# davxy/ark-ec-vrfs

Hardware: AMD Instinct MI355X
Metric: Bandersnatch IETF-ECVRF verifies/sec, 2^20 batch per GPU (higher is better)
Workload: dtype u32; 1 GPU; IETF ECVRF verify, Bandersnatch_SHA-512_ELL2, batch 2^20 per GPU, compressed points (161 B/verify), checked decode: on curve + prime-order subgroup, as arkworks' deserialisation, ad="", about 1 in 16 proofs forged (BASELINE.json configs[2]); global_batch=1048576, parallelism=items sharded x1, result gather only, subgroup_check=True

## Files before the change

ark_ec_vrfs_amd/csrc/api.hip:

```cpp
#include "../../include/vrfhip.h"

#include <hip/hip_runtime.h>

#include <algorithm>
#include <cstdio>
#include <cstdlib>
#include <cstring>
#include <memory>
#include <mutex>
#include <string>
#include <thread>
#include <vector>

#include "kernels.h"
#include "digest.cuh"
#include "msm.cuh"
#include "msm_g1.h"
#include "p256.h"
#include "bsw.h"
#include "constants_bsw.gen.h"

namespace vrf {
size_t pairing_oct_lines_bytes(size_t items);
void launch_pairing_check2_oct_split(size_t n, const uint8_t* g1, const uint8_t* g2, size_t g2_stride, uint8_t* status, void* ws,
// ... 131 lines not shown
  int prev = -1;
  bool ok = true;
  explicit DeviceGuard(int dev) {
    if (hipGetDevice(&prev) != hipSuccess) prev = -1;
    if (prev != dev) ok = hipSetDevice(dev) == hipSuccess;
  }
  ~DeviceGuard() {
    if (prev >= 0) (void)hipSetDevice(prev);
  }
};

int32_t alloc_workspace(vrfhip_ctx* ctx, size_t cap) {
  if (ctx->d_ws) {
    HIP_TRY(hipFree(ctx->d_ws));
    ctx->d_ws = nullptr;
    ctx->ws_cap = 0;
    ctx->ws_bytes = 0;
  }
  if (ctx->sw) {
    const size_t total = p256::ws_bytes(cap);
    HIP_TRY(hipMalloc(&ctx->d_ws, total));
    ctx->p256_ws = p256::ws_carve(ctx->d_ws, cap);
    ctx->ws_cap = cap;
    ctx->ws_bytes = total;
    return VRFHIP_SUCCESS;
  }
  size_t tabs_b = cap * WS_TABS * WIN_TABLE_WORDS * sizeof(uint32_t);
  size_t pts_b = cap * PROVE_PTS_WORDS * sizeof(uint32_t);
  size_t aux_b = cap * AUX_WORDS * sizeof(uint32_t);
  size_t flags_b = (cap + 255) & ~size_t(255);
  size_t total = tabs_b + pts_b + aux_b + flags_b;
  HIP_TRY(hipMalloc(&ctx->d_ws, total));
  uint8_t* p = static_cast<uint8_t*>(ctx->d_ws);
  ctx->ws.tabs = reinterpret_cast<uint32_t*>(p); p += tabs_b;
  ctx->ws.pts = reinterpret_cast<uint32_t*>(p); p += pts_b;
  ctx->ws.aux = reinterpret_cast<uint32_t*>(p); p += aux_b;
  ctx->ws.flags = p;
  ctx->ws_cap = cap;
  ctx->ws_bytes = total;
  return VRFHIP_SUCCESS;
}

int32_t ensure_workspace(vrfhip_ctx* ctx, size_t items) {
  size_t want = std::min(items, ctx->chunk_limit);
  if (want <= ctx->ws_cap) return VRFHIP_SUCCESS;
  return alloc_workspace(ctx, want);
}

int32_t ensure_stage(vrfhip_ctx* ctx, size_t bytes) {
  if (bytes <= ctx->stage_bytes) return VRFHIP_SUCCESS;
  if (ctx->d_stage) {
    HIP_TRY(hipMemset(ctx->d_stage, 0, ctx->stage_bytes));
    HIP_TRY(hipFree(ctx->d_stage));
    ctx->d_stage = nullptr;
    ctx->stage_bytes = 0;
  }
  HIP_TRY(hipMalloc(&ctx->d_stage, bytes));
  ctx->stage_bytes = bytes;
  return VRFHIP_SUCCESS;
}

int32_t ensure_msm_workspace(vrfhip_ctx* ctx, size_t need) {
  if (need <= ctx->msm_ws_bytes) return VRFHIP_SUCCESS;
  if (ctx->d_msm_ws) HIP_TRY(hipFree(ctx->d_msm_ws));
  ctx->d_msm_ws = nullptr;
  ctx->msm_ws_bytes = 0;
// ... 2996 lines not shown
```

ark_ec_vrfs_amd/csrc/fr.cuh:

```cuda
#pragma once
#include "fe.cuh"

VRF_NS_BEGIN

template <class C>
VRF_HD void fr_montmul(uint32_t out[8], const uint32_t a[8], const uint32_t b[8]) {
  uint32_t t[10];
#pragma unroll
  for (int i = 0; i < 10; ++i) t[i] = 0;
#pragma unroll
  for (int i = 0; i < 8; ++i) {
    uint64_t c = 0;
#pragma unroll
    for (int j = 0; j < 8; ++j) {
      uint64_t x = (uint64_t)a[j] * b[i] + t[j] + c;
      t[j] = (uint32_t)x;
      c = x >> 32;
    }
    uint64_t x = (uint64_t)t[8] + c;
    t[8] = (uint32_t)x;
    t[9] = (uint32_t)(x >> 32);
    uint32_t m = t[0] * C::R_NINV32;
    c = ((uint64_t)m * C::r32(0) + t[0]) >> 32;
#pragma unroll
// ... 187 lines not shown
  acc5_muladd(v2, c2, vrfk::BS_GLV_B2_MAG, !(vrfk::BS_GLV_C2_NEG ^ vrfk::BS_GLV_B2_NEG));
  k1 = glv_finish(v1);
  k2 = glv_finish(v2);
}
#endif

VRF_HD void scalar_recode_signed4_128(uint32_t out[4], const uint32_t k[4]) {
  uint32_t c = 0;
#pragma unroll
  for (int i = 0; i < 4; ++i) {
    uint64_t x = (uint64_t)k[i] + 0x88888888u + c;
    out[i] = (uint32_t)x;
    c = (uint32_t)(x >> 32);
  }
}
VRF_HD int scalar_digit4_128(const uint32_t rec[4], int w) {
  uint32_t word = rec[0];
#pragma unroll
  for (int i = 1; i < 4; ++i)
    if ((w >> 3) == i) word = rec[i];
  return (int)((word >> ((w & 7) * 4)) & 15u) - 8;
}

constexpr uint32_t GLV_HALF_TOP_WORD_CAP = 0x77777777u;
static_assert(GLV_HALF_TOP_WORD_CAP < 0x80000000u, "bit 127 of a GLV half must be clear: the joint ladders start at bit 126");

VRF_HD int scalar_bit_128(const uint32_t k[4], int bit) {
  uint32_t word = k[0];
#pragma unroll
  for (int i = 1; i < 4; ++i)
    if ((bit >> 5) == i) word = k[i];
  return (int)((word >> (bit & 31)) & 1u);
}
VRF_HD void scalar_recode_signed2_128(uint32_t out[4], const uint32_t k[4]) {
  uint32_t c = 0;
#pragma unroll
  for (int i = 0; i < 4; ++i) {
    uint64_t x = (uint64_t)k[i] + 0x55555555u + c;
    out[i] = (uint32_t)x;
    c = (uint32_t)(x >> 32);
  }
}
VRF_HD int scalar_digit2_128(const uint32_t rec[4], int w) {
  uint32_t word = rec[0];
#pragma unroll
  for (int i = 1; i < 4; ++i)
    if ((w >> 4) == i) word = rec[i];
  return (int)((word >> ((w & 15) * 2)) & 3u) - 1;
}

VRF_NS_END
```

ark_ec_vrfs_amd/csrc/k_verify.hip:

```cpp
#include "kernels.h"
#include "tai_find.cuh"

VRF_NS_BEGIN


template <class S, int MINW>
__global__ void __launch_bounds__(BLOCK, MINW) k_verify_decode(VerifyArgs a) {
  size_t first = ((size_t)blockIdx.x * BLOCK + threadIdx.x) * a.k_decode;
  if (first >= a.n) return;
  verify_decode_multi<S, 3, false, S::HAS_GLV>(a.k_decode, a.T, first, a.n, a.pk, a.h, a.gamma, a.ws.tabs, a.ws.pts, a.ws.flags,
                                               a.check_mask, a.c, a.s);
}

template <class S>
__global__ void __launch_bounds__(BLOCK, 2) k_verify_input_from_alpha(size_t n, BytesView msg, uint8_t* enc, uint32_t* tabs,
                                                                      DevTables T, const uint8_t* tai_ctr) {
  size_t i = (size_t)blockIdx.x * BLOCK + threadIdx.x;
  if (i >= n) return;
  const uint8_t* m; uint32_t len;
  bytes_get(msg, i, m, len);
  PtE h = data_to_point<S>(m, len, T.sq, tai_ctr ? tai_ctr[i] : 0u);
  FeN x, y;
  te_to_affine(x, y, h);
  uint32_t e[8];
  te_encode_affine(e, x, y, T.sq.str.flags);
  store32(enc, i, e);
  if constexpr (S::HAS_GLV) jt_park_xy(tabs + i * (VERIFY_TABS * WIN_TABLE_WORDS) + JT_HXY, x, y);
  else build_glv_tables<S>(tabs + i * (VERIFY_TABS * WIN_TABLE_WORDS) + 2 * WIN_TABLE_WORDS, x, y);
}
template <class S, int MINW>
__global__ void __launch_bounds__(BLOCK, MINW) k_verify_decode_skip_h(VerifyArgs a) {
  size_t first = ((size_t)blockIdx.x * BLOCK + threadIdx.x) * a.k_decode;
  if (first >= a.n) return;
  verify_decode_multi<S, 2, true, S::HAS_GLV>(a.k_decode, a.T, first, a.n, a.pk, nullptr, a.gamma, a.ws.tabs, a.ws.pts,
                                              a.ws.flags, a.check_mask, a.c, a.s);
}

template <class S, int MINW>
__global__ void __launch_bounds__(BLOCK, MINW) k_verify_decode_keyed(VerifyArgs a) {
  size_t first = ((size_t)blockIdx.x * BLOCK + threadIdx.x) * a.k_decode;
  if (first >= a.n) return;
  verify_decode_multi<S, 2, false, S::HAS_GLV>(a.k_decode, a.T, first, a.n, nullptr, a.h, a.gamma, a.ws.tabs, a.ws.pts,
                                               a.ws.flags, a.check_mask, a.c, a.s);
#pragma unroll 1
  for (int k = 0; k < a.k_decode; ++k) {
    const size_t i = first + k;
    if (i >= a.n) break;
    const uint32_t key = a.key_index[i];
    const bool key_ok = key < a.n_keys && a.key_valid[key] != 0;
    if (!key_ok) a.ws.flags[i] = 0;
  }
}

template <class S>
__global__ void __launch_bounds__(BLOCK) k_verify_comb_u(VerifyArgs a) {
  size_t i = (size_t)blockIdx.x * BLOCK + threadIdx.x;
  if (i >= a.n) return;
  uint32_t c[8], s[8];
  load32(c, a.c, i); load32(s, a.s, i);
  load_cs_reduced<S>(c, s);
  const uint32_t key = a.key_index[i] < a.n_keys ? a.key_index[i] : 0;
  PtE r = gcomb_mul<S>(a.T.g_comb, s);
  r = comb_add<S>(r, a.key_combs + (size_t)key * COMB_WORDS, c, true);
  uint32_t* out = a.ws.pts + i * PROVE_PTS_WORDS;
  fe_store(out, r.X); fe_store(out + NL, r.Y); fe_store(out + 2 * NL, r.Z);
}

template <class S>
__global__ void __launch_bounds__(BLOCK) k_verify_decode_affine(VerifyArgs a) {
  size_t i = (size_t)blockIdx.x * BLOCK + threadIdx.x;
  if (i >= a.n) return;
  uint32_t xy[3][16], enc[3][8];
  const uint32_t* p0 = reinterpret_cast<const uint32_t*>(a.pk + i * 64);
  const uint32_t* p1 = reinterpret_cast<const uint32_t*>(a.h + i * 64);
  const uint32_t* p2 = reinterpret_cast<const uint32_t*>(a.gamma + i * 64);
#pragma unroll
  for (int j = 0; j < 16; ++j) { xy[0][j] = p0[j]; xy[1][j] = p1[j]; xy[2][j] = p2[j]; }
  uint32_t c[8], s[8];
  if constexpr (S::HAS_GLV) {
    load32(c, a.c, i); load32(s, a.s, i);
    load_cs_reduced<S>(c, s);
  }
  bool ok = verify_decode_affine_item<S, S::HAS_GLV>(enc, xy, a.ws.tabs + i * (VERIFY_TABS * WIN_TABLE_WORDS), a.T.sq,
                                                     a.check_mask, a.affine_in == 2, c, s);
  uint32_t* aux = a.ws.aux + i * AUX_WORDS;
#pragma unroll
  for (int j = 0; j < 8; ++j) { aux[j] = enc[0][j]; aux[8 + j] = enc[1][j]; aux[16 + j] = enc[2][j]; }
  a.ws.flags[i] = ok ? 1 : 0;
}

template <class S, int HALF>
__global__ void __launch_bounds__(BLOCK) k_verify_straus(VerifyArgs a) {
  size_t i = (size_t)blockIdx.x * BLOCK + threadIdx.x;
  if (i >= a.n) return;
  uint32_t c[8], s[8];
  load32(c, a.c, i); load32(s, a.s, i);
  load_cs_reduced<S>(c, s);
  uint32_t* out = a.ws.pts + i * PROVE_PTS_WORDS + HALF * UV_WORDS;
  const uint32_t* tabs = a.ws.tabs + i * (VERIFY_TABS * WIN_TABLE_WORDS);
  if constexpr (S::HAS_GLV) verify_joint_item<S, HALF>(out, a.T, tabs, c, s);
  else verify_straus_item<S, HALF>(out, a.T, tabs, c, s);
}

template <class S>
__global__ void __launch_bounds__(BLOCK) k_verify_straus_both(VerifyArgs a) {
  size_t i = (size_t)blockIdx.x * BLOCK + threadIdx.x;
  if (i >= a.n) return;
  uint32_t c[8], s[8];
  load32(c, a.c, i); load32(s, a.s, i);
  load_cs_reduced<S>(c, s);
  const uint32_t* tabs = a.ws.tabs + i * (VERIFY_TABS * WIN_TABLE_WORDS);
  if constexpr (S::HAS_GLV) {
    if (blockIdx.y == 0) verify_joint_item<S, 1>(a.ws.pts + i * PROVE_PTS_WORDS + UV_WORDS, a.T, tabs, c, s);
    else verify_joint_item<S, 0>(a.ws.pts + i * PROVE_PTS_WORDS, a.T, tabs, c, s);
  } else {
    if (blockIdx.y == 0) verify_straus_item<S, 1>(a.ws.pts + i * PROVE_PTS_WORDS + UV_WORDS, a.T, tabs, c, s);
    else verify_straus_item<S, 0>(a.ws.pts + i * PROVE_PTS_WORDS, a.T, tabs, c, s);
  }
}

template <class S, int MINW>
__global__ void __launch_bounds__(BLOCK, MINW) k_verify_finish(VerifyArgs a) {
  size_t first = ((size_t)blockIdx.x * BLOCK + threadIdx.x) * a.k_lane;
  if (first >= a.n) return;
  verify_finish_multi<S>(a.k_lane, first, a.n, a.ws.pts, PROVE_PTS_WORDS, a.pk, a.h, a.gamma,
                         a.affine_in ? a.ws.aux : nullptr, AUX_WORDS, a.c, a.s, a.ad, a.ws.flags, a.status,
                         a.T.sq.str, a.key_index, a.n_keys);
}

template <class S>
static void launch_verify_t(const VerifyArgs& a_in, hipStream_t st, hipEvent_t* ev) {
  VerifyArgs a = a_in;
  if (a.k_decode <= 0) a.k_decode = a.k_lane;
  const size_t lanes_k_ = (a.n + a.k_lane - 1) / a.k_lane;
  const dim3 gk = grid_for(lanes_k_);
  const size_t lanes_d = (a.n + a.k_decode - 1) / a.k_decode;
  const dim3 gd = grid_for(lanes_d);
  if (ev) (void)hipEventRecord(ev[0], st);
  if (a.key_index) VRF_LAUNCH_MINW(k_verify_decode_keyed, S, lanes_d, gd, spread_lds_bytes(gd.x), st, a);
  else if (a.h_in_tabs) VRF_LAUNCH_MINW(k_verify_decode_skip_h, S, lanes_d, gd, spread_lds_bytes(gd.x), st, a);
  else if (a.affine_in) hipLaunchKernelGGL(k_verify_decode_affine<S>, grid_for(a.n), dim3(BLOCK), 0, st, a);
  else VRF_LAUNCH_MINW(k_verify_decode, S, lanes_d, gd, spread_lds_bytes(gd.x), st, a);
  if (!ev && !a.key_index && a.n <= STRAUS_FUSE_MAX_ITEMS) {
    dim3 g2 = grid_for(a.n);
    g2.y = 2;
    hipLaunchKernelGGL(k_verify_straus_both<S>, g2, dim3(BLOCK), 0, st, a);
    if (a.u_out) { launch_test_verify_uv_readout(a, st); return; }
// ... 31 lines not shown
```

ark_ec_vrfs_amd/csrc/te.cuh:

```cuda
#pragma once
#include "fe.cuh"

VRF_NS_BEGIN

#if VRF_FIELD == 0
struct CurveBS {
  static constexpr int ANEG = 5;
  static constexpr bool A_PLUS_ONE = false;
  static constexpr int COFACTOR_LOG2 = 2;
  static VRF_HD FeN d() { return fe_const(vrfk::BS_D_M); }
  static VRF_HD FeN aneg_m() { return fe_const(vrfk::FIVE_M); }
  static VRF_HD FeN gx() { return fe_const(vrfk::BS_GX_M); }
  static VRF_HD FeN gy() { return fe_const(vrfk::BS_GY_M); }
  static VRF_HD FeN bx() { return fe_const(vrfk::BS_BX_M); }
  static VRF_HD FeN by() { return fe_const(vrfk::BS_BY_M); }
  template <int L, int V>
  static VRF_HD Fe<5 * L, 5 * V> mul_aneg(const Fe<L, V>& a) { return fe_mul5(a); }
  static VRF_HD uint32_t r32(int i) { return vrfk::BS_R32[i]; }
  static VRF_HD uint32_t r_r1(int i) { return vrfk::BS_R_R1[i]; }
  static VRF_HD uint32_t r_r2(int i) { return vrfk::BS_R_R2[i]; }
  static constexpr uint32_t R_NINV32 = vrfk::BS_R_NINV32;
};

struct CurveJJ {
// ... 151 lines not shown
  auto D = fe_mul<CHAIN>(p.Z, q.Z);
  auto E = fe_mul2<CHAIN>(p.X, q.Y, p.Y, X2);
  auto H = te_add_h<C, CHAIN>(p.X, p.Y, q.X, neg, q.Y);
  auto F = fe_sub(D, Cc);
  auto G = fe_add(D, Cc);
  PtE r;
  r.X = fe_mul<CHAIN>(E, F);
  r.Y = fe_mul<CHAIN>(G, H);
  r.Z = fe_mul<CHAIN>(F, G);
  r.T = fe_zero();
  if (need_t) r.T = fe_mul<CHAIN>(E, H);
  return r;
}

struct PtA {
  FeN x, y, dt;
};
constexpr int PTA_WORDS = 3 * NL;
VRF_HD PtA pta_load(const uint32_t* m) {
  PtA a;
  a.x = fe_load<1, 2>(m); a.y = fe_load<1, 2>(m + NL); a.dt = fe_load<1, 2>(m + 2 * NL);
  return a;
}
VRF_HD void pta_store(uint32_t* m, const PtA& a) {
  fe_store(m, a.x); fe_store(m + NL, a.y); fe_store(m + 2 * NL, a.dt);
}
VRF_HD PtA pta_identity() {
  PtA a;
  a.x = fe_zero(); a.y = fe_one(); a.dt = fe_zero();
  return a;
}

template <class C, bool CHAIN = false>
VRF_HD PtE te_add_affine(const PtE& p, const PtA& q, bool neg) {
  auto X2 = fe_cneg(neg, q.x);
  auto dT2 = fe_cneg(neg, q.dt);
  auto Cc = fe_mul<CHAIN>(p.T, dT2);
  auto E = fe_mul2<CHAIN>(p.X, q.y, p.Y, X2);
  auto H = te_add_h<C, CHAIN>(p.X, p.Y, q.x, neg, q.y);
  auto F = fe_sub(p.Z, Cc);
  auto G = fe_add(p.Z, Cc);
  PtE r;
  r.X = fe_mul<CHAIN>(E, F);
  r.Y = fe_mul<CHAIN>(G, H);
  r.Z = fe_mul<CHAIN>(F, G);
  r.T = fe_mul<CHAIN>(E, H);
  return r;
}

#if VRF_FIELD == 0
template <class C>
VRF_HD PtE te_psi(const PtE& p) {
  const FeN b = fe_const(vrfk::BS_PSI_B_M), c = fe_const(vrfk::BS_PSI_C_M);
  auto YY = fe_sqr(p.Y);
  auto ZZ = fe_sqr(p.Z);
  auto XY = fe_mul(p.X, p.Y);
  auto bZZ = fe_mul(ZZ, b);
  auto A = fe_sub(ZZ, YY);
  auto Bv = fe_sub(YY, bZZ);
  auto Cv = fe_add(YY, bZZ);
  auto cA = fe_mul(A, c);
  auto bC = fe_mul(Cv, b);
  PtE r;
  r.X = fe_mul(cA, Bv);
  r.Y = fe_mul(bC, XY);
  r.Z = fe_mul(XY, Bv);
  r.T = fe_mul(cA, bC);
  bool exc = fe_is_zero(r.Z);
  PtE id = te_identity();
  r.X = fe_select(exc, id.X, r.X);
  r.Y = fe_select(exc, id.Y, r.Y);
  r.Z = fe_select(exc, id.Z, r.Z);
  r.T = fe_select(exc, id.T, r.T);
  return r;
}

#else
template <class C>
VRF_HD PtE te_psi(const PtE& p);
// ... 36 lines not shown
```

ark_ec_vrfs_amd/csrc/vrf_core.cuh:

```cuda
#pragma once
#include "fe.cuh"
#include "fr.cuh"
#include "sha512.cuh"
#include "te.cuh"

VRF_NS_BEGIN

enum : uint32_t { ST_OK = 0, ST_VERIFICATION_FAILURE = 1, ST_INVALID_DATA = 2 };


constexpr int WIN_ENTRIES = 8;
constexpr int WIN_TABLE_WORDS = WIN_ENTRIES * PTC_WORDS;

enum : int { SUBGROUP_2DESCENT = 0, SUBGROUP_TATE8 = 1, SUBGROUP_ORDER = 2, SUBGROUP_HALVE_TATE4 = 3 };

#if VRF_FIELD == 0
struct SuiteBS : CurveBS {
  static constexpr bool HAS_GLV = true;
  static constexpr int SUBGROUP = SUBGROUP_2DESCENT;
  static constexpr bool H2C_ELL2 = true;
};

struct SuiteJJ : CurveJJ {
  static constexpr bool HAS_GLV = false;
// ... 69 lines not shown
  else den = fe_canon(fe_add(fe_mul(y2, C::d()), C::aneg_m()));
  bool dz = true;
#pragma unroll
  for (int i = 0; i < NL; ++i) dz = dz && (den.v[i] == 0);
  r.ok = r.ok && !dz;
  r.den = fe_select(dz, fe_one(), den);
  return r;
}
VRF_HD bool decode_finish_x(Fe<1, 4>& x_out, const DecodeA& a, const FeN& root, bool sq, const SqrtTables& T) {
  uint32_t xw[8];
  fe_to_u256(xw, root);
  uint32_t nz = 0;
#pragma unroll
  for (int i = 0; i < 8; ++i) nz |= xw[i];
  sq = sq || (nz == 0);
  bool greater = te_x_sign(xw, T.str.flags);
  x_out = fe_norm(fe_cneg(greater != a.flag, root));
  if ((T.str.flags & SS_SIGN_PARITY) && nz == 0 && a.flag) sq = false;
  return a.ok && sq;
}
template <class C>
VRF_HD bool decode_phase_b(Fe<1, 4>& x_out, const DecodeA& a, const FeN& den_inv, const SqrtTables& T) {
  FeN w = fe_mul(a.num, den_inv);
  FeN root;
  bool sq = fe_sqrt_or_zsqrt(root, w, T);
  return decode_finish_x(x_out, a, root, sq, T);
}
template <class C>
VRF_HD bool decode_by_inv_root(Fe<1, 4>& x_out, const DecodeA& a, const SqrtTables& T) {
  FeN ir;
  const bool sq = fe_inv_sqrt(ir, fe_mul(a.num, a.den), T);
  return decode_finish_x(x_out, a, fe_mul(a.num, ir), sq, T);
}

#if VRF_FIELD == 0
template <class S>
VRF_HD bool subgroup_by_2descent(const FeN& y, const SqrtTables& T) {
  const FeN one = fe_one();
  const bool is_identity = fe_eq(y, one);
  const auto omy = fe_norm(fe_sub(one, y));
  const FeN t1 = fe_mul(fe_mul(omy, fe_add(one, y)), fe_const(vrfk::BS_DESC_B_M));
  const auto lin = fe_norm(fe_add(fe_mul(y, fe_const(vrfk::BS_DESC_1PE2_M)), fe_const(vrfk::BS_DESC_1ME2_M)));
  const FeN t2 = fe_mul(fe_mul(omy, lin), fe_const(vrfk::BS_DESC_B_M));
  const bool s1 = fe_is_nonzero_square(t1, T);
  const bool s2 = fe_is_nonzero_square(t2, T);
  return is_identity || (s1 && s2);
}
#endif

enum : uint32_t { CHK_PUBLIC = 1, CHK_INPUT = 2, CHK_OUTPUT = 4, CHK_PROOF = 8,
                  CHK_CT_TABLES = 0x100 };

template <class C>
VRF_HD void build_win_table_from(uint32_t* tab, PtE acc) {
  PtC c1 = te_to_cached<C>(acc);
  ptc_store(tab, c1);
#pragma unroll 1
  for (int j = 1; j < WIN_ENTRIES; ++j) {
    acc = te_add_cached<C>(acc, c1, false);
    ptc_store(tab + j * PTC_WORDS, te_to_cached<C>(acc));
  }
}
template <class C>
VRF_HD void build_glv_tables(uint32_t* tab, const FeP& x, const FeP& y) {
  PtE p = te_from_affine(x, y);
  if constexpr (!C::HAS_GLV) {
// ... 470 lines not shown
    for (int j = 0; j < 8; ++j) out[j] = c[j];
  } else {
    fr_reduce256<S>(out, c);
  }
}

template <class S>
VRF_HD bool challenge_supplied(uint32_t out[8], const uint32_t c[8], const SuiteStr& ss) {
  const bool fits = u256_fits_bytes(c, ss.challenge_len);
  uint32_t cr[8];
  fr_reduce256<S>(cr, c);
#pragma unroll
  for (int j = 0; j < 8; ++j) out[j] = fits ? cr[j] : 0u;
  return fits;
}

constexpr int UV_WORDS = 3 * NL;

VRF_HD FeN fe_sel3(int p, const FeN& a, const FeN& b, const FeN& c) {
  return fe_select(p == 0, a, fe_select(p == 1, b, c));
}

constexpr int VERIFY_TABS = 6;

template <class S>
VRF_HD void load_cs_reduced(uint32_t c[8], uint32_t s[8]) {
  uint32_t cr[8];
  fr_reduce256<S>(cr, c);
  const bool s_ok = fr_is_canonical<S>(s);
#pragma unroll
  for (int j = 0; j < 8; ++j) { c[j] = s_ok ? cr[j] : 0u; s[j] = s_ok ? s[j] : 0u; }
}

constexpr int JT_Y_ENTRIES = 12, JT_V_ENTRIES = 15;
constexpr int JT_Y = 0;
constexpr int JT_V = JT_Y + JT_Y_ENTRIES * PTC_WORDS;
constexpr int JT_EXT = JT_V + JT_V_ENTRIES * PTC_WORDS;
constexpr int JT_YEXT = JT_EXT + 8 * PTC_WORDS;
constexpr int JT_HXY = JT_YEXT + 2 * PTC_WORDS;
constexpr int JT_GXY = JT_HXY + 2 * NL;
static_assert(JT_GXY + 2 * NL <= VERIFY_TABS * WIN_TABLE_WORDS, "the joint tables and their parking fit the item's region");

VRF_HD void pte_store(uint32_t* m, const PtE& p) {
  fe_store(m, p.X); fe_store(m + NL, p.Y); fe_store(m + 2 * NL, p.Z); fe_store(m + 3 * NL, p.T);
}
VRF_HD PtE pte_load(const uint32_t* m) {
  PtE p;
  p.X = fe_load<1, 5>(m); p.Y = fe_load<1, 5>(m + NL); p.Z = fe_load<1, 5>(m + 2 * NL); p.T = fe_load<1, 5>(m + 3 * NL);
  return p;
}
VRF_HD void jt_park_xy(uint32_t* m, const Fe<1, 4>& x, const FeN& y) { fe_store(m, x); fe_store(m + NL, y); }

#if VRF_FIELD == 0
template <class C>
VRF_HD PtE te_psi_signed(const PtE& p, bool neg) {
  const FeN b = fe_const(vrfk::BS_PSI_B_M);
  const auto c = fe_norm(fe_cneg(neg, fe_const(vrfk::BS_PSI_C_M)));
  auto YY = fe_sqr(p.Y);
  auto ZZ = fe_sqr(p.Z);
  auto XY = fe_mul(p.X, p.Y);
  auto bZZ = fe_mul(ZZ, b);
  auto A = fe_sub(ZZ, YY);
  auto Bv = fe_sub(YY, bZZ);
  auto Cv = fe_add(YY, bZZ);
  auto cA = fe_mul(A, c);
  auto bC = fe_mul(Cv, b);
  PtE r;
  r.X = fe_mul(cA, Bv);
  r.Y = fe_mul(bC, XY);
  r.Z = fe_mul(XY, Bv);
  r.T = fe_mul(cA, bC);
  bool exc = fe_is_zero(r.Z);
  PtE id = te_identity();
  r.X = fe_select(exc, id.X, r.X);
// ... 38 lines not shown
}

template <class S>
VRF_HD void build_joint_v_table(uint32_t* reg, const uint32_t c[8], const uint32_t s[8]) {
  GlvHalf h[4];
  glv_decompose_bs(h[0], h[1], c);
  glv_decompose_bs(h[2], h[3], s);
  const bool neg0 = !h[0].neg, neg1 = !h[1].neg, neg2 = h[2].neg, neg3 = h[3].neg;
#pragma unroll 1
  for (int p = 0; p < 2; ++p) {
    const uint32_t* xy = reg + (p == 0 ? JT_GXY : JT_HXY);
    const bool nb = p == 0 ? neg0 : neg2, npsi = p == 0 ? neg1 : neg3;
    const FeN x = fe_mul(fe_cneg(nb, fe_load<1, 4>(xy)), fe_one());
    const PtE b = te_from_affine(x, fe_load<1, 2>(xy + NL));
    const PtE q = te_psi_signed<S>(b, nb != npsi);
    const int m = 1 << (2 * p);
    ptc_store(reg + JT_V + (m - 1) * PTC_WORDS, te_to_cached<S>(b));
    ptc_store(reg + JT_V + (2 * m - 1) * PTC_WORDS, te_to_cached<S>(q));
    pte_store(reg + JT_EXT + (m - 1) * PTC_WORDS, b);
    pte_store(reg + JT_EXT + (2 * m - 1) * PTC_WORDS, q);
  }
#pragma unroll 1
  for (int m = 3; m < 16; ++m) {
    if ((m & (m - 1)) == 0) continue;
    const int top = m >= 8 ? 8 : (m >= 4 ? 4 : 2);
    const PtE e = te_add_cached<S>(pte_load(reg + JT_EXT + (m - top - 1) * PTC_WORDS),
                                   ptc_load(reg + JT_V + (top - 1) * PTC_WORDS), false);
    ptc_store(reg + JT_V + (m - 1) * PTC_WORDS, te_to_cached<S>(e));
    if (m < 8) pte_store(reg + JT_EXT + (m - 1) * PTC_WORDS, e);
  }
}

template <class S>
VRF_HD bool verify_decode_item(const DevTables& T, const uint32_t pk[8], const uint32_t hh[8],
                               const uint32_t gamma[8], uint32_t* tabs, uint32_t check_mask = 0) {
  DecodeA a0 = decode_phase_a<S>(pk), a1 = decode_phase_a<S>(hh), a2 = decode_phase_a<S>(gamma);
  FeN dens[3] = {a0.den, a1.den, a2.den}, dinv[3];
  fe_batch_inv(dinv, dens);
  bool valid = true;
#pragma unroll 1
  for (int p = 0; p < 3; ++p) {
    DecodeA a;
    a.y = fe_sel3(p, a0.y, a1.y, a2.y);
    a.den = fe_sel3(p, a0.den, a1.den, a2.den);
    a.num = fe_select(p == 0, a0.num, fe_select(p == 1, a1.num, a2.num));
    a.flag = p == 0 ? a0.flag : (p == 1 ? a1.flag : a2.flag);
    a.ok = p == 0 ? a0.ok : (p == 1 ? a1.ok : a2.ok);
    FeN di = fe_sel3(p, dinv[0], dinv[1], dinv[2]);
    Fe<1, 4> x;
    valid = decode_phase_b<S>(x, a, di, T.sq) && valid;
    build_glv_tables<S>(tabs + p * 2 * WIN_TABLE_WORDS, x, a.y);
    if ((check_mask >> p) & 1u) valid = in_prime_subgroup<S>(fe_mul(x, fe_one()), a.y, T.sq) && valid;
  }
  return valid;
}

constexpr int VERIFY_K = 8;
constexpr int DEC_SLOT = 4 * NL;

template <class S, int NP = 3, bool SKIP_H = false, bool JOINT = false>
VRF_HD void verify_decode_multi(int K, const DevTables& T, size_t first, size_t n, const uint8_t* pk,
                                const uint8_t* hh, const uint8_t* gamma, uint32_t* tabs_base,
                                uint32_t* scratch_base, uint8_t* flags, uint32_t check_mask = 0,
                                const uint8_t* c_arr = nullptr, const uint8_t* s_arr = nullptr) {
  (void)scratch_base;
  uint32_t valid_mask = 0xffffffffu;
#pragma unroll 1
  for (int j = NP * K - 1; j >= 0; --j) {
    const size_t item = first + j / NP;
    const int p = SKIP_H ? (j % NP) * 2 : j % NP + (3 - NP);
    if (item < n) {
      const uint8_t* src = p == 0 ? pk : (p == 1 ? hh : gamma);
      uint32_t enc[8];
      const uint32_t* w = reinterpret_cast<const uint32_t*>(src + item * 32);
#pragma unroll
      for (int k = 0; k < 8; ++k) enc[k] = w[k];
      const DecodeA a = decode_phase_a<S>(enc);
      Fe<1, 4> x;
      bool ok = decode_by_inv_root<S>(x, a, T.sq);
      if constexpr (JOINT) {
        uint32_t* reg = tabs_base + item * (VERIFY_TABS * WIN_TABLE_WORDS);
        if (p == 0) build_joint_y_table<S>(reg, x, a.y);
        else jt_park_xy(reg + (p == 1 ? JT_HXY : JT_GXY), x, a.y);
        if (p == (SKIP_H ? 2 : 1)) {
          uint32_t c[8], s[8];
          const uint32_t* wc = reinterpret_cast<const uint32_t*>(c_arr + item * 32);
          const uint32_t* ws = reinterpret_cast<const uint32_t*>(s_arr + item * 32);
#pragma unroll
          for (int k = 0; k < 8; ++k) { c[k] = wc[k]; s[k] = ws[k]; }
          load_cs_reduced<S>(c, s);
          build_joint_v_table<S>(reg, c, s);
        }
      } else {
        uint32_t* tab = tabs_base + item * (VERIFY_TABS * WIN_TABLE_WORDS) + p * 2 * WIN_TABLE_WORDS;
        build_glv_tables<S>(tab, x, a.y);
      }
      if ((check_mask >> p) & 1u) ok = in_prime_subgroup<S>(fe_mul(x, fe_one()), a.y, T.sq) && ok;
      if (!ok) valid_mask &= ~(1u << (j / NP));
    }
  }
#pragma unroll 1
  for (int k = 0; k < K; ++k)
    if (first + k < n) flags[first + k] = (valid_mask >> k) & 1;
}

template <class S>
VRF_HD void verify_finish_multi(int K, size_t first, size_t n, uint32_t* pts_base, int pts_stride,
                                const uint8_t* pk, const uint8_t* hh, const uint8_t* gamma,
                                const uint32_t* enc_aux, int aux_stride, const uint8_t* c_arr,
                                const uint8_t* s_arr, const BytesViewLite& ad, const uint8_t* flags,
                                uint8_t* status, const SuiteStr& ss, const uint32_t* key_index = nullptr,
                                size_t n_keys = 0) {
  FeN run = fe_one();
#pragma unroll 1
  for (int j = 0; j < 2 * K; ++j) {
    const size_t item = first + j / 2;
    if (item < n) {
      uint32_t* slot = pts_base + item * pts_stride;
      FeP z = fe_load<1, 5>(slot + (j & 1) * UV_WORDS + 2 * NL);
      fe_store(slot + 2 * UV_WORDS + (j & 1) * NL, run);
      run = fe_mul(run, z);
    }
  }
  FeN inv = fe_inv(run);
  uint32_t encv[8];
#pragma unroll
// ... 17 lines not shown
        uint32_t pts[5][8], c[8], sc[8];
        if (enc_aux) {
          const uint32_t* aux = enc_aux + item * aux_stride;
#pragma unroll
          for (int k = 0; k < 8; ++k) { pts[0][k] = aux[k]; pts[1][k] = aux[8 + k]; pts[2][k] = aux[16 + k]; }
        } else {
          size_t pk_row = item;
          if (key_index) pk_row = key_index[item] < n_keys ? key_index[item] : 0;
          const uint32_t* w0 = reinterpret_cast<const uint32_t*>(pk + pk_row * 32);
          const uint32_t* w1 = reinterpret_cast<const uint32_t*>(hh + item * 32);
          const uint32_t* w2 = reinterpret_cast<const uint32_t*>(gamma + item * 32);
#pragma unroll
          for (int k = 0; k < 8; ++k) { pts[0][k] = w0[k]; pts[1][k] = w1[k]; pts[2][k] = w2[k]; }
        }
        const uint32_t* wc = reinterpret_cast<const uint32_t*>(c_arr + item * 32);
        const uint32_t* ws = reinterpret_cast<const uint32_t*>(s_arr + item * 32);
#pragma unroll
        for (int k = 0; k < 8; ++k) { pts[3][k] = e[k]; pts[4][k] = encv[k]; c[k] = wc[k]; sc[k] = ws[k]; }
        const uint8_t* adp; uint32_t adl;
        bytes_lite_get(ad, item, adp, adl);
        uint32_t c2[8], cr[8];
        challenge5<S>(c2, pts, adp, adl, ss);
        proof_challenge_decode<S>(cr, c, ss);
        uint32_t diff = 0;
#pragma unroll
        for (int k = 0; k < 8; ++k) diff |= c2[k] ^ cr[k];
        bool valid = flags[item] != 0 && fr_is_canonical<S>(sc);
        status[item] = (uint8_t)(!valid ? ST_INVALID_DATA : (diff == 0 ? ST_OK : ST_VERIFICATION_FAILURE));
      }
    }
  }
}

template <class S, bool JOINT = false>
VRF_HD bool verify_decode_affine_item(uint32_t enc_out[3][8], const uint32_t (&xy)[3][16], uint32_t* tabs,
                                      const SqrtTables& T, uint32_t check_mask = 0, bool mont256 = false,
                                      const uint32_t* c = nullptr, const uint32_t* s = nullptr) {
  bool valid = true;
#pragma unroll 1
  for (int p = 0; p < 3; ++p) {
    uint32_t xin[8], yin[8], xw[8], yw[8];
#pragma unroll
    for (int j = 0; j < 8; ++j) {
      xin[j] = p == 0 ? xy[0][j] : p == 1 ? xy[1][j] : xy[2][j];
      yin[j] = p == 0 ? xy[0][8 + j] : p == 1 ? xy[1][8 + j] : xy[2][8 + j];
    }
    valid = valid && !u256_ge(xin, vrfk::Q32) && !u256_ge(yin, vrfk::Q32);
    FeN x = fe_from_abi(xw, xin, mont256), y = fe_from_abi(yw, yin, mont256);
    FeN x2 = fe_sqr(x), y2 = fe_sqr(y), xyv = fe_mul(x, y);
    auto lhs = te_curve_lhs<S>(x2, y2);
    valid = fe_eq(lhs, fe_mul(fe_mul(fe_sqr(xyv), S::d()), fe_one())) && valid;
    if constexpr (JOINT) {
      if (p == 0) build_joint_y_table<S>(tabs, x, y);
      else jt_park_xy(tabs + (p == 1 ? JT_HXY : JT_GXY), x, y);
    } else {
      build_glv_tables<S>(tabs + p * 2 * WIN_TABLE_WORDS, x, y);
    }
    if ((check_mask >> p) & 1u) valid = in_prime_subgroup<S>(x, y, T) && valid;
    uint32_t e[8];
#pragma unroll
    for (int j = 0; j < 8; ++j) e[j] = yw[j];
    if (te_x_sign(xw, T.str.flags)) e[7] |= 0x80000000u;
#pragma unroll
    for (int j = 0; j < 8; ++j) {
      if (p == 0) enc_out[0][j] = e[j];
      if (p == 1) enc_out[1][j] = e[j];
      if (p == 2) enc_out[2][j] = e[j];
    }
  }
  if constexpr (JOINT) build_joint_v_table<S>(tabs, c, s);
  return valid;
}

template <class S, int HALF>
VRF_HD void verify_straus_item(uint32_t* out_uv, const DevTables& T, const uint32_t* tabs,
                               const uint32_t c[8], const uint32_t s[8]) {
  if constexpr (!S::HAS_GLV) {
    uint32_t recs[8], recc[8];
    scalar_recode_signed4(recs, s);
    scalar_recode_signed4(recc, c);
    PtE r;
    if (HALF == 0) {
      r = win_mul<S, false, true>(tabs, recc, true, challenge_top_window(T.sq.str));
      r = gcomb_add<S, true>(r, T.g_comb, s);
    } else {
      r = straus2<S, true>(tabs + 2 * WIN_TABLE_WORDS, recs, tabs + 4 * WIN_TABLE_WORDS, recc, true, challenge_top_window(T.sq.str));
    }
    fe_store(out_uv, r.X);
    fe_store(out_uv + NL, r.Y);
    fe_store(out_uv + 2 * NL, r.Z);
    return;
  } else {
  Straus4 q;
  GlvHalf h[4];
  glv_decompose_bs(h[0], h[1], c);
#pragma unroll
  for (int t = 0; t < 2; ++t) {
    scalar_recode_signed4_128(q.rec[t], h[t].mag);
    q.neg[t] = !h[t].neg;
  }
  PtE r;
  if (HALF == 0) {
    q.tab[0] = tabs; q.tab[1] = tabs + WIN_TABLE_WORDS;
// ... 26 lines not shown
  scalar_recode_signed2_128(r1, c1.mag);
  scalar_recode_signed2_128(r2, c2.mag);
  const bool n1 = !c1.neg, n2 = !c2.neg;
  PtE acc = te_identity();
#pragma unroll 1
  for (int w = 63; w >= 0; --w) {
    if (w != 63) {
#pragma unroll 1
      for (int j = 0; j < 2; ++j) acc = te_dbl<S, true>(acc, j == 1);
    }
    const int d1 = scalar_digit2_128(r1, w), d2 = scalar_digit2_128(r2, w);
    bool neg;
    const int idx = joint_y_index(n1 ? -d1 : d1, n2 ? -d2 : d2, neg);
    acc = te_add_cached<S, true>(acc, win_lookup(ytab, idx), neg, w == 0);
  }
  return acc;
}
VRF_HD int joint_v_index(const uint32_t (&m)[4][4], int bit) {
  return scalar_bit_128(m[0], bit) | (scalar_bit_128(m[1], bit) << 1) | (scalar_bit_128(m[2], bit) << 2) |
         (scalar_bit_128(m[3], bit) << 3);
}
template <class S>
VRF_HD PtE joint_v_ladder(const uint32_t* vtab, const uint32_t (&m)[4][4]) {
  const PtC first = win_lookup(vtab, joint_v_index(m, 126));
  PtE acc;
  acc.X = first.X; acc.Y = first.Y; acc.Z = first.Z; acc.T = fe_zero();
#pragma unroll 1
  for (int bit = 125; bit >= 0; --bit) {
    acc = te_dbl<S, true>(acc, true);
    acc = te_add_cached<S, true>(acc, win_lookup(vtab, joint_v_index(m, bit)), false, false);
  }
  return acc;
}
template <class S, int HALF>
VRF_HD void verify_joint_item(uint32_t* out_uv, const DevTables& T, const uint32_t* reg, const uint32_t c[8],
                              const uint32_t s[8]) {
  GlvHalf h[4];
  glv_decompose_bs(h[0], h[1], c);
  PtE r;
  if (HALF == 0) {
    r = joint_u_ladder<S>(reg + JT_Y, h[0], h[1]);
    r = gcomb_add<S, true>(r, T.g_comb, s);
  } else {
    glv_decompose_bs(h[2], h[3], s);
    uint32_t m[4][4];
#pragma unroll
    for (int t = 0; t < 4; ++t)
#pragma unroll
      for (int i = 0; i < 4; ++i) m[t][i] = h[t].mag[i];
    r = joint_v_ladder<S>(reg + JT_V, m);
  }
  fe_store(out_uv, r.X);
  fe_store(out_uv + NL, r.Y);
  fe_store(out_uv + 2 * NL, r.Z);
}

template <class S>
VRF_HD uint32_t verify_finish_item(const uint32_t* uv, const uint32_t pk[8], const uint32_t hh[8],
                                   const uint32_t gamma[8], const uint32_t c[8],
                                   const uint32_t s[8], bool valid, const uint8_t* ad,
                                   uint32_t ad_len, const SuiteStr& ss) {
  valid = valid && fr_is_canonical<S>(s);
  uint32_t cr[8];
  proof_challenge_decode<S>(cr, c, ss);
  FeP zin[2] = {fe_load<1, 5>(uv + 2 * NL), fe_load<1, 5>(uv + UV_WORDS + 2 * NL)};
  FeN zi[2];
  fe_batch_inv(zi, zin);
  uint32_t pts[5][8];
#pragma unroll
  for (int i = 0; i < 8; ++i) { pts[0][i] = pk[i]; pts[1][i] = hh[i]; pts[2][i] = gamma[i]; }
  te_encode_affine(pts[3], fe_mul(fe_load<1, 5>(uv), zi[0]), fe_mul(fe_load<1, 5>(uv + NL), zi[0]), ss.flags);
  te_encode_affine(pts[4], fe_mul(fe_load<1, 5>(uv + UV_WORDS), zi[1]),
                   fe_mul(fe_load<1, 5>(uv + UV_WORDS + NL), zi[1]), ss.flags);
  uint32_t c2[8];
  challenge5<S>(c2, pts, ad, ad_len, ss);
  uint32_t diff = 0;
#pragma unroll
  for (int i = 0; i < 8; ++i) diff |= c2[i] ^ cr[i];
  if (!valid) return ST_INVALID_DATA;
  return diff == 0 ? ST_OK : ST_VERIFICATION_FAILURE;
}

VRF_HD void put_dst_prime(Sha512& h, const SuiteStr& ss) { sha512_put_packed(h, ss.dst_prime_w, ss.dst_prime_len); }
// ... 767 lines not shown
```

Measured before the change: 30.80 million verifies/s.

## Use affine sign-aligned 8-entry table for the joint V ladder

Replaces the 15-entry cached-coordinate table of the 4-scalar joint V ladder with an 8-entry affine table under a sign-aligned column recoding, so each step is a mixed addition with a sign flip. The table is normalised with a batched inversion, and in the default path that inversion rides on the decode inverse-square-root, costing a few extra multiplies instead of a separate inversion. Each entry sits in one 128-byte line, which cuts table size and per-step multiplies and skips the unneeded T coordinate on the final add. In exchange, table build gains extra work and the workspace layout and parking offsets change.

```diff
diff --git a/ark_ec_vrfs_amd/csrc/api.hip b/ark_ec_vrfs_amd/csrc/api.hip
--- a/ark_ec_vrfs_amd/csrc/api.hip
+++ b/ark_ec_vrfs_amd/csrc/api.hip
@@ -187,6 +187,7 @@
   size_t total = tabs_b + pts_b + aux_b + flags_b;
   HIP_TRY(hipMalloc(&ctx->d_ws, total));
   uint8_t* p = static_cast<uint8_t*>(ctx->d_ws);
+  static_assert((WS_TABS * WIN_TABLE_WORDS * sizeof(uint32_t)) % 128 == 0, "an item's table region is whole 128-byte lines");
   ctx->ws.tabs = reinterpret_cast<uint32_t*>(p); p += tabs_b;
   ctx->ws.pts = reinterpret_cast<uint32_t*>(p); p += pts_b;
   ctx->ws.aux = reinterpret_cast<uint32_t*>(p); p += aux_b;
diff --git a/ark_ec_vrfs_amd/csrc/fr.cuh b/ark_ec_vrfs_amd/csrc/fr.cuh
--- a/ark_ec_vrfs_amd/csrc/fr.cuh
+++ b/ark_ec_vrfs_amd/csrc/fr.cuh
@@ -243,6 +243,32 @@
     if ((bit >> 5) == i) word = k[i];
   return (int)((word >> (bit & 31)) & 1u);
 }
+struct SacV {
+  uint32_t sgn[4];
+  uint32_t u[3][4];
+  bool fix;
+};
+VRF_HD void glv_recode_sac(SacV& r, const uint32_t (&m)[4][4]) {
+  r.fix = (m[0][0] & 1u) == 0;
+#pragma unroll
+  for (int i = 0; i < 4; ++i) r.sgn[i] = ~((m[0][i] >> 1) | (i < 3 ? m[0][i + 1] << 31 : 0u));
+  r.sgn[3] &= 0x7fffffffu;
+#pragma unroll
+  for (int j = 0; j < 3; ++j) {
+    uint32_t c = 0;
+#pragma unroll
+    for (int i = 0; i < 4; ++i) {
+      const uint64_t x = (uint64_t)m[j + 1][i] + r.sgn[i] + c;
+      r.u[j][i] = (uint32_t)x ^ r.sgn[i];
+      c = (uint32_t)(x >> 32);
+    }
+  }
+}
+VRF_HD int sac_index(const SacV& r, int bit) {
+  return scalar_bit_128(r.u[0], bit) | (scalar_bit_128(r.u[1], bit) << 1) | (scalar_bit_128(r.u[2], bit) << 2);
+}
+VRF_HD bool sac_neg(const SacV& r, int bit) { return scalar_bit_128(r.sgn, bit) != 0; }
+
 VRF_HD void scalar_recode_signed2_128(uint32_t out[4], const uint32_t k[4]) {
   uint32_t c = 0;
 #pragma unroll
diff --git a/ark_ec_vrfs_amd/csrc/k_verify.hip b/ark_ec_vrfs_amd/csrc/k_verify.hip
--- a/ark_ec_vrfs_amd/csrc/k_verify.hip
+++ b/ark_ec_vrfs_amd/csrc/k_verify.hip
@@ -8,7 +8,7 @@
 __global__ void __launch_bounds__(BLOCK, MINW) k_verify_decode(VerifyArgs a) {
   size_t first = ((size_t)blockIdx.x * BLOCK + threadIdx.x) * a.k_decode;
   if (first >= a.n) return;
-  verify_decode_multi<S, 3, false, S::HAS_GLV>(a.k_decode, a.T, first, a.n, a.pk, a.h, a.gamma, a.ws.tabs, a.ws.pts, a.ws.flags,
+  verify_decode_multi<S, 3, false, S::HAS_GLV, S::HAS_GLV>(a.k_decode, a.T, first, a.n, a.pk, a.h, a.gamma, a.ws.tabs, a.ws.pts, a.ws.flags,
                                                a.check_mask, a.c, a.s);
 }
 
@@ -32,7 +32,7 @@
 __global__ void __launch_bounds__(BLOCK, MINW) k_verify_decode_skip_h(VerifyArgs a) {
   size_t first = ((size_t)blockIdx.x * BLOCK + threadIdx.x) * a.k_decode;
   if (first >= a.n) return;
-  verify_decode_multi<S, 2, true, S::HAS_GLV>(a.k_decode, a.T, first, a.n, a.pk, nullptr, a.gamma, a.ws.tabs, a.ws.pts,
+  verify_decode_multi<S, 2, true, S::HAS_GLV, S::HAS_GLV>(a.k_decode, a.T, first, a.n, a.pk, nullptr, a.gamma, a.ws.tabs, a.ws.pts,
                                               a.ws.flags, a.check_mask, a.c, a.s);
 }
 
@@ -40,7 +40,7 @@
 __global__ void __launch_bounds__(BLOCK, MINW) k_verify_decode_keyed(VerifyArgs a) {
   size_t first = ((size_t)blockIdx.x * BLOCK + threadIdx.x) * a.k_decode;
   if (first >= a.n) return;
-  verify_decode_multi<S, 2, false, S::HAS_GLV>(a.k_decode, a.T, first, a.n, nullptr, a.h, a.gamma, a.ws.tabs, a.ws.pts,
+  verify_decode_multi<S, 2, false, S::HAS_GLV, S::HAS_GLV>(a.k_decode, a.T, first, a.n, nullptr, a.h, a.gamma, a.ws.tabs, a.ws.pts,
                                                a.ws.flags, a.check_mask, a.c, a.s);
 #pragma unroll 1
   for (int k = 0; k < a.k_decode; ++k) {
@@ -81,7 +81,7 @@
     load32(c, a.c, i); load32(s, a.s, i);
     load_cs_reduced<S>(c, s);
   }
-  bool ok = verify_decode_affine_item<S, S::HAS_GLV>(enc, xy, a.ws.tabs + i * (VERIFY_TABS * WIN_TABLE_WORDS), a.T.sq,
+  bool ok = verify_decode_affine_item<S, S::HAS_GLV, S::HAS_GLV>(enc, xy, a.ws.tabs + i * (VERIFY_TABS * WIN_TABLE_WORDS), a.T.sq,
                                                      a.check_mask, a.affine_in == 2, c, s);
   uint32_t* aux = a.ws.aux + i * AUX_WORDS;
 #pragma unroll
@@ -98,7 +98,7 @@
   load_cs_reduced<S>(c, s);
   uint32_t* out = a.ws.pts + i * PROVE_PTS_WORDS + HALF * UV_WORDS;
   const uint32_t* tabs = a.ws.tabs + i * (VERIFY_TABS * WIN_TABLE_WORDS);
-  if constexpr (S::HAS_GLV) verify_joint_item<S, HALF>(out, a.T, tabs, c, s);
+  if constexpr (S::HAS_GLV) verify_joint_item<S, HALF, true>(out, a.T, tabs, c, s);
   else verify_straus_item<S, HALF>(out, a.T, tabs, c, s);
 }
 
@@ -111,8 +111,8 @@
   load_cs_reduced<S>(c, s);
   const uint32_t* tabs = a.ws.tabs + i * (VERIFY_TABS * WIN_TABLE_WORDS);
   if constexpr (S::HAS_GLV) {
-    if (blockIdx.y == 0) verify_joint_item<S, 1>(a.ws.pts + i * PROVE_PTS_WORDS + UV_WORDS, a.T, tabs, c, s);
-    else verify_joint_item<S, 0>(a.ws.pts + i * PROVE_PTS_WORDS, a.T, tabs, c, s);
+    if (blockIdx.y == 0) verify_joint_item<S, 1, true>(a.ws.pts + i * PROVE_PTS_WORDS + UV_WORDS, a.T, tabs, c, s);
+    else verify_joint_item<S, 0, true>(a.ws.pts + i * PROVE_PTS_WORDS, a.T, tabs, c, s);
   } else {
     if (blockIdx.y == 0) verify_straus_item<S, 1>(a.ws.pts + i * PROVE_PTS_WORDS + UV_WORDS, a.T, tabs, c, s);
     else verify_straus_item<S, 0>(a.ws.pts + i * PROVE_PTS_WORDS, a.T, tabs, c, s);
diff --git a/ark_ec_vrfs_amd/csrc/te.cuh b/ark_ec_vrfs_amd/csrc/te.cuh
--- a/ark_ec_vrfs_amd/csrc/te.cuh
+++ b/ark_ec_vrfs_amd/csrc/te.cuh
@@ -207,7 +207,7 @@
 }
 
 template <class C, bool CHAIN = false>
-VRF_HD PtE te_add_affine(const PtE& p, const PtA& q, bool neg) {
+VRF_HD PtE te_add_affine(const PtE& p, const PtA& q, bool neg, bool need_t = true) {
   auto X2 = fe_cneg(neg, q.x);
   auto dT2 = fe_cneg(neg, q.dt);
   auto Cc = fe_mul<CHAIN>(p.T, dT2);
@@ -219,7 +219,8 @@
   r.X = fe_mul<CHAIN>(E, F);
   r.Y = fe_mul<CHAIN>(G, H);
   r.Z = fe_mul<CHAIN>(F, G);
-  r.T = fe_mul<CHAIN>(E, H);
+  r.T = fe_zero();
+  if (need_t) r.T = fe_mul<CHAIN>(E, H);
   return r;
 }
 
diff --git a/ark_ec_vrfs_amd/csrc/vrf_core.cuh b/ark_ec_vrfs_amd/csrc/vrf_core.cuh
--- a/ark_ec_vrfs_amd/csrc/vrf_core.cuh
+++ b/ark_ec_vrfs_amd/csrc/vrf_core.cuh
@@ -125,6 +125,22 @@
   const bool sq = fe_inv_sqrt(ir, fe_mul(a.num, a.den), T);
   return decode_finish_x(x_out, a, fe_mul(a.num, ir), sq, T);
 }
+template <class C>
+VRF_HD bool decode_by_inv_root_ride(Fe<1, 4>& x_out, FeN& pinv, bool ride, const FeN& P, const DecodeA& a, const SqrtTables& T) {
+  FeN w = fe_mul(a.num, a.den), m = w;
+  if (ride) {
+    m = fe_select(fe_is_zero(w), fe_one(), w);
+    w = fe_mul(m, fe_sqr(P));
+  }
+  FeN ir;
+  const bool sq = fe_inv_sqrt(ir, w, T);
+  if (ride) {
+    const FeN rp = fe_mul(ir, P);
+    pinv = fe_mul(fe_mul(ir, m), rp);
+    ir = rp;
+  }
+  return decode_finish_x(x_out, a, fe_mul(a.num, ir), sq, T);
+}
 
 #if VRF_FIELD == 0
 template <class S>
@@ -661,14 +677,23 @@
   for (int j = 0; j < 8; ++j) { c[j] = s_ok ? cr[j] : 0u; s[j] = s_ok ? s[j] : 0u; }
 }
 
-constexpr int JT_Y_ENTRIES = 12, JT_V_ENTRIES = 15;
+constexpr int JT_Y_ENTRIES = 12, JT_VA_ENTRIES = 8, JT_V_ENTRIES = 15;
+constexpr int JT_VA_STRIDE = 32;
 constexpr int JT_Y = 0;
-constexpr int JT_V = JT_Y + JT_Y_ENTRIES * PTC_WORDS;
-constexpr int JT_EXT = JT_V + JT_V_ENTRIES * PTC_WORDS;
-constexpr int JT_YEXT = JT_EXT + 8 * PTC_WORDS;
+constexpr int JT_VA = 448;
+constexpr int JT_VEXT = JT_VA + JT_VA_ENTRIES * JT_VA_STRIDE;
+constexpr int JT_YEXT = JT_VEXT + JT_VA_ENTRIES * PTC_WORDS;
 constexpr int JT_HXY = JT_YEXT + 2 * PTC_WORDS;
 constexpr int JT_GXY = JT_HXY + 2 * NL;
-static_assert(JT_GXY + 2 * NL <= VERIFY_TABS * WIN_TABLE_WORDS, "the joint tables and their parking fit the item's region");
+constexpr int JT_VPFX = JT_GXY + 2 * NL;
+constexpr int JT_V = JT_VA;
+constexpr int JT_EXT = JT_VPFX;
+static_assert(JT_VA >= JT_Y + JT_Y_ENTRIES * PTC_WORDS && JT_VA % 32 == 0 && PTA_WORDS <= JT_VA_STRIDE &&
+              (VERIFY_TABS * WIN_TABLE_WORDS) % 32 == 0, "a V entry is one 128-byte line of a 128-byte aligned region");
+static_assert(3 * PTC_WORDS <= (JT_VA_ENTRIES - 1) * JT_VA_STRIDE, "the cached bases are parked behind entry 0 of JT_VA");
+static_assert(JT_VPFX + JT_VA_ENTRIES * NL <= VERIFY_TABS * WIN_TABLE_WORDS, "the joint tables and their parking fit the item's region");
+static_assert(JT_V + JT_V_ENTRIES * PTC_WORDS <= JT_YEXT && JT_EXT >= JT_GXY + 2 * NL && JT_EXT + 8 * PTC_WORDS <= VERIFY_TABS * WIN_TABLE_WORDS,
+              "the cached form of V's table keeps clear of JT_Y, JT_YEXT and the parked points");
 
 VRF_HD void pte_store(uint32_t* m, const PtE& p) {
   fe_store(m, p.X); fe_store(m + NL, p.Y); fe_store(m + 2 * NL, p.Z); fe_store(m + 3 * NL, p.T);
@@ -773,6 +798,55 @@
 }
 
 template <class S>
+VRF_HD void build_joint_va_table(uint32_t* reg, const uint32_t c[8], const uint32_t s[8]) {
+  GlvHalf h[4];
+  glv_decompose_bs(h[0], h[1], c);
+  glv_decompose_bs(h[2], h[3], s);
+  const bool neg0 = !h[0].neg, neg1 = !h[1].neg, neg2 = h[2].neg, neg3 = h[3].neg;
+#pragma unroll 1
+  for (int p = 0; p < 2; ++p) {
+    const uint32_t* xy = reg + (p == 0 ? JT_GXY : JT_HXY);
+    const bool nb = p == 0 ? neg0 : neg2, npsi = p == 0 ? neg1 : neg3;
+    const FeN x = fe_mul(fe_cneg(nb, fe_load<1, 4>(xy)), fe_one());
+    const PtE b = te_from_affine(x, fe_load<1, 2>(xy + NL));
+    const PtE q = te_psi_signed<S>(b, nb != npsi);
+    const PtC bc = te_to_cached<S>(b);
+    if (p == 0) {
+      PtA a;
+      a.x = x; a.y = fe_load<1, 2>(xy + NL); a.dt = bc.dT;
+      pta_store(reg + JT_VA, a);
+      pte_store(reg + JT_VEXT, b);
+    } else {
+      ptc_store(reg + JT_VA + JT_VA_STRIDE + PTC_WORDS, bc);
+    }
+    ptc_store(reg + JT_VA + JT_VA_STRIDE + 2 * p * PTC_WORDS, te_to_cached<S>(q));
+  }
+  FeN run = fe_one();
+#pragma unroll 1
+  for (int u = 1; u < JT_VA_ENTRIES; ++u) {
+    const int hb = u >= 4 ? 2 : (u >= 2 ? 1 : 0);
+    const PtE e = te_add_cached<S>(pte_load(reg + JT_VEXT + (u - (1 << hb)) * PTC_WORDS),
+                                   ptc_load(reg + JT_VA + JT_VA_STRIDE + hb * PTC_WORDS), false);
+    pte_store(reg + JT_VEXT + u * PTC_WORDS, e);
+    fe_store(reg + JT_VPFX + u * NL, run);
+    run = fe_mul(run, e.Z);
+  }
+  fe_store(reg + JT_VPFX, run);
+}
+template <class S>
+VRF_HD void joint_va_normalise(uint32_t* reg, FeN inv) {
+#pragma unroll 1
+  for (int u = JT_VA_ENTRIES - 1; u >= 1; --u) {
+    const PtE e = pte_load(reg + JT_VEXT + u * PTC_WORDS);
+    const FeN zi = fe_mul(inv, fe_load<1, 2>(reg + JT_VPFX + u * NL));
+    inv = fe_mul(inv, e.Z);
+    PtA a;
+    a.x = fe_mul(e.X, zi); a.y = fe_mul(e.Y, zi); a.dt = fe_mul(fe_mul(e.T, zi), S::d());
+    pta_store(reg + JT_VA + u * JT_VA_STRIDE, a);
+  }
+}
+
+template <class S>
 VRF_HD bool verify_decode_item(const DevTables& T, const uint32_t pk[8], const uint32_t hh[8],
                                const uint32_t gamma[8], uint32_t* tabs, uint32_t check_mask = 0) {
   DecodeA a0 = decode_phase_a<S>(pk), a1 = decode_phase_a<S>(hh), a2 = decode_phase_a<S>(gamma);
@@ -799,7 +873,7 @@
 constexpr int VERIFY_K = 8;
 constexpr int DEC_SLOT = 4 * NL;
 
-template <class S, int NP = 3, bool SKIP_H = false, bool JOINT = false>
+template <class S, int NP = 3, bool SKIP_H = false, bool JOINT = false, bool VA = false>
 VRF_HD void verify_decode_multi(int K, const DevTables& T, size_t first, size_t n, const uint8_t* pk,
                                 const uint8_t* hh, const uint8_t* gamma, uint32_t* tabs_base,
                                 uint32_t* scratch_base, uint8_t* flags, uint32_t check_mask = 0,
@@ -818,9 +892,15 @@
       for (int k = 0; k < 8; ++k) enc[k] = w[k];
       const DecodeA a = decode_phase_a<S>(enc);
       Fe<1, 4> x;
-      bool ok = decode_by_inv_root<S>(x, a, T.sq);
+      bool ok;
       if constexpr (JOINT) {
+        constexpr bool RIDE = VA && (NP == 3 || SKIP_H);
         uint32_t* reg = tabs_base + item * (VERIFY_TABS * WIN_TABLE_WORDS);
+        const bool ride = RIDE && p == 0;
+        FeN P = fe_one(), pinv = fe_zero();
+        if (ride) P = fe_load<1, 2>(reg + JT_VPFX);
+        ok = decode_by_inv_root_ride<S>(x, pinv, ride, P, a, T.sq);
+        if (ride) joint_va_normalise<S>(reg, pinv);
         if (p == 0) build_joint_y_table<S>(reg, x, a.y);
         else jt_park_xy(reg + (p == 1 ? JT_HXY : JT_GXY), x, a.y);
         if (p == (SKIP_H ? 2 : 1)) {
@@ -830,9 +910,15 @@
 #pragma unroll
           for (int k = 0; k < 8; ++k) { c[k] = wc[k]; s[k] = ws[k]; }
           load_cs_reduced<S>(c, s);
-          build_joint_v_table<S>(reg, c, s);
+          if constexpr (VA) {
+            build_joint_va_table<S>(reg, c, s);
+            if constexpr (!RIDE) joint_va_normalise<S>(reg, fe_inv(fe_load<1, 2>(reg + JT_VPFX)));
+          } else {
+            build_joint_v_table<S>(reg, c, s);
+          }
         }
       } else {
+        ok = decode_by_inv_root<S>(x, a, T.sq);
         uint32_t* tab = tabs_base + item * (VERIFY_TABS * WIN_TABLE_WORDS) + p * 2 * WIN_TABLE_WORDS;
         build_glv_tables<S>(tab, x, a.y);
       }
@@ -916,7 +1002,7 @@
   }
 }
 
-template <class S, bool JOINT = false>
+template <class S, bool JOINT = false, bool VA = false>
 VRF_HD bool verify_decode_affine_item(uint32_t enc_out[3][8], const uint32_t (&xy)[3][16], uint32_t* tabs,
                                       const SqrtTables& T, uint32_t check_mask = 0, bool mont256 = false,
                                       const uint32_t* c = nullptr, const uint32_t* s = nullptr) {
@@ -952,7 +1038,12 @@
       if (p == 2) enc_out[2][j] = e[j];
     }
   }
-  if constexpr (JOINT) build_joint_v_table<S>(tabs, c, s);
+  if constexpr (JOINT && VA) {
+    build_joint_va_table<S>(tabs, c, s);
+    joint_va_normalise<S>(tabs, fe_inv(fe_load<1, 2>(tabs + JT_VPFX)));
+  } else if constexpr (JOINT) {
+    build_joint_v_table<S>(tabs, c, s);
+  }
   return valid;
 }
 
@@ -1045,7 +1136,23 @@
   }
   return acc;
 }
-template <class S, int HALF>
+template <class S>
+VRF_HD PtE joint_va_ladder(const uint32_t* vtab, const uint32_t (&m)[4][4]) {
+  SacV r;
+  glv_recode_sac(r, m);
+  const PtA first = pta_load(vtab + sac_index(r, 127) * JT_VA_STRIDE);
+  PtE acc;
+  acc.X = first.x; acc.Y = first.y; acc.Z = fe_one(); acc.T = fe_zero();
+#pragma unroll 1
+  for (int bit = 126; bit >= 0; --bit) {
+    acc = te_dbl<S, true>(acc, true);
+    acc = te_add_affine<S, true>(acc, pta_load(vtab + sac_index(r, bit) * JT_VA_STRIDE), sac_neg(r, bit), bit == 0);
+  }
+  const PtE fixed = te_add_affine<S, true>(acc, pta_load(vtab), true, false);
+  acc.X = fe_select(r.fix, fixed.X, acc.X); acc.Y = fe_select(r.fix, fixed.Y, acc.Y); acc.Z = fe_select(r.fix, fixed.Z, acc.Z);
+  return acc;
+}
+template <class S, int HALF, bool VA = false>
 VRF_HD void verify_joint_item(uint32_t* out_uv, const DevTables& T, const uint32_t* reg, const uint32_t c[8],
                               const uint32_t s[8]) {
   GlvHalf h[4];
@@ -1061,7 +1168,8 @@
     for (int t = 0; t < 4; ++t)
 #pragma unroll
       for (int i = 0; i < 4; ++i) m[t][i] = h[t].mag[i];
-    r = joint_v_ladder<S>(reg + JT_V, m);
+    if constexpr (VA) r = joint_va_ladder<S>(reg + JT_VA, m);
+    else r = joint_v_ladder<S>(reg + JT_V, m);
   }
   fe_store(out_uv, r.X);
   fe_store(out_uv + NL, r.Y);
```

New measurement: 31.96 million verifies/s (median of 6 runs). 1.04x the previous value.
